# sekelle/SPH-EXA

Hardware: AMD Instinct MI355X
Metric: particle-updates/sec (whole node), Sedov -n 400 and Evrard+gravity -n 200 (higher is better)
Workload: dtype fp64 coordinates + fp32 hydro (reference precision mix); 1 GPU; model=sedov -n 400 --prop ve (64000000 particles), global_batch=64000000, seq_len=1, parallelism=sfc-domain-decomposition x1, ranks=1, backend=none, leaf_capacity=512

## Files before the change

### sphexa_amd/csrc/hip/hydro.hip

```cpp
#include <cfloat>
#include <cstdlib>
#include <type_traits>

#include "common.h"
#include "hip_api.h"
#include "sphx/sph_math.hpp"
#include "staged.h"

namespace sphx::hip
{

#ifndef SPHX_PAIR_BLOCK
#define SPHX_PAIR_BLOCK 256
#endif
constexpr int kBlock = SPHX_PAIR_BLOCK;

template<int B = kBlock>
__device__ __forceinline__ bool targetOf(const NbrArgs& a, int64_t& i, PackedLane& pl, unsigned& n)
{
    __shared__ uint32_t ctabAll[B / 64][kChunkCap];
    unsigned lb     = xcdRemap(blockIdx.x, gridDim.x);
    int64_t t       = int64_t(lb) * B + threadIdx.x;
    i               = a.first + t;
    const int64_t g = t >> 6;
// ... 58 lines not shown
#define SPHX_MOM_BUF 1
#endif
static bool g_kernelFixed = SPHX_KERNEL_FIXED, g_momBuf = SPHX_MOM_BUF;
void setPairPaths(bool kernelFixed, bool momBuf)
{
    g_kernelFixed = kernelFixed;
    g_momBuf      = momBuf;
}

template<class F>
inline void withKf(const SphConsts& sc, F&& f)
{
    if (g_kernelFixed && sc.kernelChoice == 0 && sc.sincIndex == 6.0f) f(std::integral_constant<int, 6>{});
    else f(std::integral_constant<int, 0>{});
}

constexpr int kBufferFormatWord = 0x00020000;

template<class R>
__device__ __forceinline__ CoopLoader<R> coopOf(const R* rec, float4* blockTile, int64_t self, const NbrArgs& a)
{
    return CoopLoader<R>{rec, waveTile<R>(blockTile), unsigned(self)};
}

inline NbrArgs withTot(NbrArgs a, int64_t ntot)
{
    a.ntot = unsigned(ntot);
    return a;
}

inline unsigned gridT(const NbrArgs& a, int block = kBlock) { return gridFor(a.last - a.first, block); }

static int g_pairBlock = kBlock;
#ifndef SPHX_AV_BLOCK
#define SPHX_AV_BLOCK 640
#endif
#ifndef SPHX_GRADH_BLOCK
#define SPHX_GRADH_BLOCK 1024
#endif
#ifndef SPHX_XMASS_BLOCK
#define SPHX_XMASS_BLOCK 1024
#endif
static const unsigned kPairMask = []
{
    const char* e = std::getenv("SPHX_PAIR_MASK");
    return e ? unsigned(std::strtoul(e, nullptr, 0)) : 31u;
}();

void setPairBlock(int block) { g_pairBlock = block == 512 ? 512 : kBlock; }

static unsigned g_staged = []
{
    const char* e = std::getenv("SPHX_STAGED");
    return e ? unsigned(std::strtoul(e, nullptr, 0)) : 12u;
}();

void setStaged(unsigned mask) { g_staged = mask; }
unsigned stagedMask() { return g_staged; }

static bool unionLoopOn(int loop)
{
    const bool big = g_pairBlock == 512 && ((kPairMask >> loop) & 1u);
    return ((g_staged >> loop) & 1u) && (big || (g_staged & 32u));
}

static unsigned* g_stagedCounters = nullptr;
void setStagedCounters(unsigned* counters) { g_stagedCounters = counters; }

#ifndef SPHX_STB_U512
#define SPHX_STB_U512 2264
#endif
#ifndef SPHX_STB_U256
#define SPHX_STB_U256 1128
#endif
template<int B>
constexpr int kUnionCap = B == 512 ? SPHX_STB_U512 : SPHX_STB_U256;
static_assert(sizeof(BlockUnionShared<8, kUnionCap<512>, 2>) * 2 <= 160 * 1024 &&
                  sizeof(BlockUnionShared<4, kUnionCap<256>, 2>) * 4 <= 160 * 1024,
              "16 waves per CU with the unions in LDS");

static bool g_listMasks = false;
void setListMasks(bool on) { g_listMasks = on; }
bool listMasksForced() { return g_listMasks; }
bool listMasksWanted() { return g_listMasks || (g_staged & 1u) || unionLoopOn(2) || unionLoopOn(3); }

inline unsigned gridStaged(const NbrArgs& a) { return unsigned((a.last - a.first + 63) / 64); }

template<class F>
inline void withPairBlock(F&& f, int loop = 0)
{
    if (g_pairBlock == 512 && ((kPairMask >> loop) & 1u)) f(std::integral_constant<int, 512>{});
    else f(std::integral_constant<int, kBlock>{});
}

template<int L, class F>
inline void withPairBlockL(F&& f, int loop)
{
    if (g_pairBlock == 512 && ((kPairMask >> loop) & 1u)) f(std::integral_constant<int, L>{});
    else f(std::integral_constant<int, kBlock>{});
}


__global__ void packPosKernel(int64_t n, const double* __restrict__ x, const double* __restrict__ y,
                              const double* __restrict__ z, const float* __restrict__ m,
                              const float* __restrict__ xm, SrcPos* __restrict__ out)
{
    int64_t i = int64_t(blockIdx.x) * blockDim.x + threadIdx.x;
    if (i >= n) return;
    SrcPos r;
    r.x    = x[i];
    r.y    = y[i];
    r.z    = z[i];
    r.m    = m[i];
    r.xm   = xm ? xm[i] : 0.f;
    out[i] = r;
}

__global__ void packIadKernel(int64_t n, const double* __restrict__ x, const double* __restrict__ y,
                              const double* __restrict__ z, const float* __restrict__ numer,
                              const float* __restrict__ denom, const float* __restrict__ vx,
                              const float* __restrict__ vy, const float* __restrict__ vz,
                              const float* __restrict__ xm, const float* __restrict__ c,
                              const float* __restrict__ divv, SrcIad* __restrict__ out)
{
    int64_t i = int64_t(blockIdx.x) * blockDim.x + threadIdx.x;
    if (i >= n) return;
    SrcIad r;
    r.x    = x[i];
    r.y    = y[i];
    r.z    = z[i];
    r.vol  = numer ? numer[i] / denom[i] : 0.f;
    r.vx   = vx ? vx[i] : 0.f;
    r.vy   = vy ? vy[i] : 0.f;
    r.vz   = vz ? vz[i] : 0.f;
    if (c) r.c = c[i];
    else r.xm = xm ? xm[i] : 0.f;
    r.divv = divv ? divv[i] : 0.f;
// ... 259 lines not shown
    const SrcPosQ pi = ld(unsigned(i));
    const float hi = h[i], hInv = 1.f / hi, h3Inv = hInv * hInv * hInv;
    const float sx = q.inv[0] * 0.25f * hInv, sy = q.inv[1] * 0.25f * hInv, sz = q.inv[2] * 0.25f * hInv;
    float rho0 = 0.f;
    withKernelFn<kKf>(sc, wh, nullptr, [&](const auto& kf) {
        float sum = 0.f;
        forEachNeighbor<SPHX_BATCH_POS>(&pl, 0, n, ld, [&](unsigned, const SrcPosQ& pj) {
            const float ux = float(int32_t(pi.x - pj.x)) * sx;
            const float uy = float(int32_t(pi.y - pj.y)) * sy;
            const float uz = float(int32_t(pi.z - pj.z)) * sz;
            sum += kf.wqIn(sqrtF(ux * ux + uy * uy + uz * uz)) * pj.m;
        });
        rho0 = pi.m + sum / kf.wqScale();
    });
    if (!valid) return;
    const float v = pi.m / (rho0 * float(sc.K) * h3Inv);
    xm[i]         = v;
    if (xmOut) xmOut[i] = SrcXmQ{pi.x, pi.y, pi.z, v};
}

template<int W, int UCAP>
__global__ __launch_bounds__(64 * W) void xmassQStagedKernel(NbrArgs a, SphConsts sc, QFrame q,
                                                             const float* __restrict__ h,
                                                             const SrcPosQ* __restrict__ rec,
                                                             const float* __restrict__ wh, float* __restrict__ xm,
                                                             SrcXmQ* __restrict__ xmOut)
{
    using Ld = StagedLoader<SrcPosQ, W, UCAP>;
    __shared__ typename Ld::Shared sh;
    int64_t i;
    StagedLane sl;
    unsigned n;
    const bool valid = stagedTargetOf<W>(a, i, sl, n);
    const Ld ld{rec, nullptr, 0.f, &sh};
    const KernelFn kf{wh, nullptr, sc.sincIndex, sc.kernelChoice};
    const SrcPosQ pi = ld(unsigned(i));
    const float hi = h[i], hInv = 1.f / hi, h3Inv = hInv * hInv * hInv;
    const float sx = q.inv[0] * 0.25f * hInv, sy = q.inv[1] * 0.25f * hInv, sz = q.inv[2] * 0.25f * hInv;
    float rho0 = 0.f;
    forEachNeighbor<SPHX_BATCH_POS>(&sl, 0, n, ld, [&](unsigned, const SrcPosQ& pj) {
        const float ux = float(int32_t(pi.x - pj.x)) * sx;
        const float uy = float(int32_t(pi.y - pj.y)) * sy;
        const float uz = float(int32_t(pi.z - pj.z)) * sz;
        rho0 += kf.wqIn(sqrtF(ux * ux + uy * uy + uz * uz)) * pj.m;
    });
    reduceAcross(ld, rho0);
    rho0 = pi.m + rho0 / kf.wqScale();
    if (!valid || threadIdx.x >= 64) return;
    const float v = pi.m / (rho0 * float(sc.K) * h3Inv);
    xm[i]         = v;
    if (xmOut) xmOut[i] = SrcXmQ{pi.x, pi.y, pi.z, v};
}

#ifndef SPHX_ST_XMASS_W
#define SPHX_ST_XMASS_W 4
#endif
#ifndef SPHX_ST_XMASS_U
#define SPHX_ST_XMASS_U 1024
#endif

struct EosOut
{
    const double* temp = nullptr;
    float *prho = nullptr, *c = nullptr, *rho = nullptr, *p = nullptr;
};

template<class R, class G, int B = kBlock, int kKf = 0>
__global__ __launch_bounds__(B) void veDefGradhKernel(NbrArgs a, SphConsts sc, G box,
                                                           const float* __restrict__ h, const R* __restrict__ rec,
                                                           const float* __restrict__ wh, const float* __restrict__ whd,
                                                           float* __restrict__ kx, float* __restrict__ gradh,
                                                           float mUniform, const float* __restrict__ vx,
                                                           const float* __restrict__ vy, const float* __restrict__ vz,
                                                           SrcIadQ* __restrict__ iadOut, EosOut eos = EosOut{})
{
    __shared__ float4 tile[B / 64 * 64 * CoopLoader<R>::S];
    int64_t i;
    PackedLane pl;
    unsigned n;
    const bool valid = targetOf<B>(a, i, pl, n);
    float k, g;
    withKernelFn<kKf>(sc, wh, whd, [&](const auto& kf)
                 { veDefGradhJLoop(unsigned(i), sc.K, box, &pl, 0, n, h[i], coopOf(rec, tile, i, a), kf, k, g, mUniform); });
    if (!valid) return;
    kx[i]    = k;
    gradh[i] = g;
    if constexpr (std::is_same_v<R, SrcXmQ>)
    {
        if (iadOut)
        {
            const SrcXmQ pi = rec[i];
            iadOut[i]       = SrcIadQ{pi.x, pi.y, pi.z, pi.xm / k, vx[i], vy[i], vz[i], pi.xm};
        }
        if (eos.temp)
        {
            const float xmi   = rec[i].xm;
            const double rhoi = double(k) * mUniform / xmi;
            double pi, ci;
            idealGasEOS(eos.temp[i], rhoi, sc.muiConst, sc.gamma, pi, ci);
            eos.prho[i] = float(pi / (double(k) * mUniform * mUniform * g));
            eos.c[i]    = float(ci);
            if (eos.rho) eos.rho[i] = float(rhoi);
            if (eos.p) eos.p[i] = float(pi);
        }
    }
}

__global__ void eosVeKernel(int64_t first, int64_t last, SphConsts sc, const double* __restrict__ temp,
                            const float* __restrict__ m, const float* __restrict__ kx, const float* __restrict__ xm,
                            const float* __restrict__ gradh, float* __restrict__ prho, float* __restrict__ c,
                            float* __restrict__ rho, float* __restrict__ p)
{
    int64_t i = first + int64_t(blockIdx.x) * blockDim.x + threadIdx.x;
    if (i >= last) return;
    double rhoi = double(kx[i]) * m[i] / xm[i];
    double pi, ci;
    idealGasEOS(temp[i], rhoi, sc.muiConst, sc.gamma, pi, ci);
    prho[i] = float(pi / (double(kx[i]) * m[i] * m[i] * gradh[i]));
    c[i]    = float(ci);
    if (rho) rho[i] = float(rhoi);
    if (p) p[i] = float(pi);
}

__global__ void eosPolytropicKernel(int64_t first, int64_t last, const float* __restrict__ kx,
                                    const float* __restrict__ xm, const float* __restrict__ m, float* __restrict__ p,
                                    float* __restrict__ c)
{
    int64_t i = first + int64_t(blockIdx.x) * blockDim.x + threadIdx.x;
    if (i >= last) return;
    double rho = double(kx[i]) * m[i] / xm[i], pi, ci;
    polytropicEOS(rho, pi, ci);
    p[i] = float(pi);
    c[i] = float(ci);
}

void eosPolytropic(int64_t first, int64_t last, const float* kx, const float* xm, const float* m, float* p, float* c,
                   hipStream_t s)
{
    if (last <= first) return;
    eosPolytropicKernel<<<gridFor(last - first, 256), 256, 0, s>>>(first, last, kx, xm, m, p, c);
    SPHX_LAUNCH_CHECK();
}

__global__ void eosStdKernel(int64_t first, int64_t last, SphConsts sc, const double* __restrict__ temp,
                             const float* __restrict__ m, float* __restrict__ rho, float* __restrict__ p,
                             float* __restrict__ c)
{
    int64_t i = first + int64_t(blockIdx.x) * blockDim.x + threadIdx.x;
    if (i >= last) return;
    double rhoi = double(m[i]) / rho[i];
    double pi, ci;
    idealGasEOS(temp[i], rhoi, sc.muiConst, sc.gamma, pi, ci);
    rho[i] = float(rhoi);
    p[i]   = float(pi);
    c[i]   = float(ci);
}

struct Six
// ... 638 lines not shown
        double V[3] = {vx[i], vy[i], vz[i]};
        q[0] += 0.5 * mi * (V[0] * V[0] + V[1] * V[1] + V[2] * V[2]);
        if (u) q[1] += u[i] * mi;
        else if (temp) q[1] += cv * temp[i] * mi;
        q[3] += mi * V[0];
        q[4] += mi * V[1];
        q[5] += mi * V[2];
        q[6] += mi * (X[1] * V[2] - X[2] * V[1]);
        q[7] += mi * (X[2] * V[0] - X[0] * V[2]);
        q[8] += mi * (X[0] * V[1] - X[1] * V[0]);
        if (nc) q[9] += double(nc[i]);
    }
    __shared__ double red[4][10];
    int w = threadIdx.x >> 6;
    for (int k = 0; k < 10; ++k)
    {
        double v = waveSum(q[k]);
        if ((threadIdx.x & 63) == 0) red[w][k] = v;
    }
    __syncthreads();
    if (threadIdx.x < 10)
    {
        double s = 0;
        for (int ww = 0; ww < int(blockDim.x >> 6); ++ww)
            s += red[ww][threadIdx.x];
        atomicAdd(&out[threadIdx.x], s);
    }
}


void packPosQ(int64_t n, const double* x, const double* y, const double* z, const float* m, const QFrame& q,
              SrcPosQ* out, hipStream_t s)
{
    if (n <= 0) return;
    packPosQKernel<<<gridFor(n, 256), 256, 0, s>>>(0, n, x, y, z, m, q, out);
    SPHX_LAUNCH_CHECK();
}

void xmass(const NbrArgs& a, const SphConsts& sc, const Box& box, int64_t ntot, const double* x, const double* y,
           const double* z, const float* h, const float* m, const float* wh, void* rec, float* xm, hipStream_t s,
           int inDone, void* xmOut)
{
    if (a.last <= a.first) return;
    if (!sc.fixedPoint)
    {
        packPosKernel<<<gridFor(ntot, 256), 256, 0, s>>>(ntot, x, y, z, m, nullptr, (SrcPos*)rec);
        xmassKernel<<<gridT(a), kBlock, 0, s>>>(withTot(a, ntot), sc, box, h, (const SrcPos*)rec, wh, xm);
    }
    else
    {
        const QFrame q = qframeOf(box, sc.fixedPoint);
        packRanges(inDone, a, ntot, [&](int64_t lo, int64_t hi)
                   { packPosQKernel<<<gridFor(hi - lo, 256), 256, 0, s>>>(lo, hi, x, y, z, m, q, (SrcPosQ*)rec); });
        if (g_staged & 1u)
        {
            xmassQStagedKernel<SPHX_ST_XMASS_W, SPHX_ST_XMASS_U><<<gridStaged(a), 64 * SPHX_ST_XMASS_W, 0, s>>>(
                withTot(a, ntot), sc, q, h, (const SrcPosQ*)rec, wh, xm, (SrcXmQ*)xmOut);
            SPHX_LAUNCH_CHECK();
            return;
        }
        withPairBlockL<SPHX_XMASS_BLOCK>([&](auto bc)
                      {
                          constexpr int B = decltype(bc)::value;
                          withKf(sc, [&](auto kk)
                                 {
                                     xmassQKernel<B, decltype(kk)::value><<<gridT(a, B), B, 0, s>>>(
                                         withTot(a, ntot), sc, q, h, (const SrcPosQ*)rec, wh, xm, (SrcXmQ*)xmOut);
                                 });
                      }, 0);
    }
    SPHX_LAUNCH_CHECK();
}

void veDefGradh(const NbrArgs& a, const SphConsts& sc, const Box& box, int64_t ntot, const double* x,
                const double* y, const double* z, const float* h, const float* m, const float* wh, const float* whd,
                const float* xm, void* rec, float* kx, float* gradh, float mUniform, hipStream_t s, int inDone,
                void* iadOut, const float* vx, const float* vy, const float* vz, const double* eosTemp,
                float* eosPrho, float* eosC, float* eosRho, float* eosP)
{
    if (a.last <= a.first) return;
    if (mUniform > 0.f && sc.fixedPoint)
    {
        const EosOut eos{eosTemp, eosPrho, eosC, eosRho, eosP};
        const QFrame q = qframeOf(box, sc.fixedPoint);
        packRanges(inDone, a, ntot, [&](int64_t lo, int64_t hi)
                   { packXmQKernel<<<gridFor(hi - lo, 256), 256, 0, s>>>(lo, hi, x, y, z, xm, q, (SrcXmQ*)rec); });
        withPairBlockL<SPHX_GRADH_BLOCK>([&](auto bc)
                      {
                          constexpr int B = decltype(bc)::value;
                          withKf(sc, [&](auto kk)
                                 {
                                     veDefGradhKernel<SrcXmQ, QFrame, B, decltype(kk)::value><<<gridT(a, B), B, 0, s>>>(
                                         withTot(a, ntot), sc, q, h, (const SrcXmQ*)rec, wh, whd, kx, gradh, mUniform,
                                         vx, vy, vz, (SrcIadQ*)iadOut, eos);
                                 });
                      }, 1);
    }
    else
    {
        packPosKernel<<<gridFor(ntot, 256), 256, 0, s>>>(ntot, x, y, z, m, xm, (SrcPos*)rec);
        veDefGradhKernel<<<gridT(a), kBlock, 0, s>>>(withTot(a, ntot), sc, box, h, (const SrcPos*)rec, wh, whd, kx,
                                                     gradh, 0.f, vx, vy, vz, nullptr);
        SPHX_LAUNCH_CHECK();
        if (eosTemp) eosVe(a.first, a.last, sc, eosTemp, m, kx, xm, gradh, eosPrho, eosC, eosRho, eosP, s);
    }
    SPHX_LAUNCH_CHECK();
}

void eosVe(int64_t first, int64_t last, const SphConsts& sc, const double* temp, const float* m, const float* kx,
           const float* xm, const float* gradh, float* prho, float* c, float* rho, float* p, hipStream_t s)
{
    if (last <= first) return;
    eosVeKernel<<<gridFor(last - first, 256), 256, 0, s>>>(first, last, sc, temp, m, kx, xm, gradh, prho, c, rho, p);
    SPHX_LAUNCH_CHECK();
}

void eosStd(int64_t first, int64_t last, const SphConsts& sc, const double* temp, const float* m, float* rho,
            float* p, float* c, hipStream_t s)
{
    if (last <= first) return;
    eosStdKernel<<<gridFor(last - first, 256), 256, 0, s>>>(first, last, sc, temp, m, rho, p, c);
    SPHX_LAUNCH_CHECK();
}

void iad(const NbrArgs& a, const SphConsts& sc, const Box& box, int64_t ntot, const double* x, const double* y,
         const double* z, const float* h, const float* wh, const float* numer, const float* denom, void* rec,
         float* const cij[6], hipStream_t s)
{
    if (a.last <= a.first) return;
    packIadKernel<<<gridFor(ntot, 256), 256, 0, s>>>(ntot, x, y, z, numer, denom, nullptr, nullptr, nullptr,
                                                     nullptr, nullptr, nullptr, (SrcIad*)rec);
    Six c;
    for (int k = 0; k < 6; ++k)
        c.p[k] = cij[k];
    iadKernel<<<gridT(a), kBlock, 0, s>>>(withTot(a, ntot), sc, box, h, (const SrcIad*)rec, wh, c);
    SPHX_LAUNCH_CHECK();
}

inline size_t momSideOffset(int64_t ntot) { return (size_t(ntot) * sizeof(SrcMomQ64) + 255) & ~size_t(255); }
// ... 265 lines not shown
```

### sphexa_amd/csrc/hip/staged.h

```cpp
#pragma once

#include "common.h"
#include "sphx/packed_list.hpp"
#include "sphx/sph_math.hpp"

namespace sphx::hip
{

constexpr int kStRows = 64;

template<int UCAP, int RC, bool kSide>
struct StagedShared
{
    float4 rec[UCAP * RC];
    float2 side[kSide ? UCAP : 1];
    uint32_t jl[UCAP];
    uint16_t pos[kStRows * 64];
    uint32_t c0[kStRows];
    uint32_t base[kStRows];
    uint32_t mlo[kStRows], mhi[kStRows];
    int win[2];
};

struct StagedLane
// ... 265 lines not shown
    if constexpr (W > 1)
    {
        float* s            = reinterpret_cast<float*>(ld.sh->rec);
        const unsigned lane = threadIdx.x & 63, w = threadIdx.x >> 6;
        __syncthreads();
        for (int k = 0; k < n; ++k)
            s[(k * W + w) * 64 + lane] = v[k];
        __syncthreads();
        for (int k = 0; k < n; ++k)
        {
            float t = s[(k * W) * 64 + lane];
#pragma unroll
            for (int ww = 1; ww < W; ++ww)
                t += s[(k * W + ww) * 64 + lane];
            v[k] = t;
        }
    }
}

template<class R, int W, int UCAP, bool kSide, class... T>
__device__ void reduceAcrossMax(const StagedLoader<R, W, UCAP, kSide>& ld, T&... v)
{
    if constexpr (W > 1)
    {
        float* s            = reinterpret_cast<float*>(ld.sh->rec);
        const unsigned lane = threadIdx.x & 63, w = threadIdx.x >> 6;
        __syncthreads();
        int k = 0;
        ((s[(k++ * W + w) * 64 + lane] = float(v)), ...);
        __syncthreads();
        k          = 0;
        auto total = [&](int kk)
        {
            float t = s[(kk * W) * 64 + lane];
#pragma unroll
            for (int ww = 1; ww < W; ++ww)
                t = fmaxf(t, s[(kk * W + ww) * 64 + lane]);
            return t;
        };
        ((v = total(k++)), ...);
    }
}


constexpr unsigned kBuSlots = 64;
constexpr uint32_t kBuEmpty = 0xFFFFFFFFu;

struct BlockLane
{
    const int32_t* tab;
    const int32_t* rowsInt;
    unsigned nch, Tc, T;
    unsigned gfirst;

    __device__ __forceinline__ int32_t rowOf(unsigned o) const
    {
        return *(const __attribute__((address_space(4))) int32_t*)(tab + 2 + o);
    }
};

template<int NG, int UCAP, int RC>
struct BlockUnionShared
{
    static constexpr int HS = 64 * NG;
    union
    {
        uint4 rec[(UCAP + 1) * RC];
        uint32_t ctab[NG][kChunkCap];
    };
    uint4 tab[HS];
    uint16_t dense[HS];
    unsigned wsum[NG];
    unsigned fail;
};

template<int B>
__device__ __forceinline__ bool blockTargetOf(const NbrArgs& a, int64_t& i, PackedLane& pl, unsigned& n, BlockLane& bl)
{
    const unsigned lb   = xcdRemap(blockIdx.x, gridDim.x);
    const int64_t t     = int64_t(lb) * B + threadIdx.x;
    i                   = a.first + t;
    const int64_t g     = t >> 6;
    const int64_t G     = (a.last - a.first + 63) / 64;
    const unsigned lane = threadIdx.x & 63;
    bl.tab              = a.nidx + g * int64_t(packedTableInts(a.ngmax));
    bl.rowsInt          = a.nidx + packedTableRegion(G, a.ngmax);
    bl.nch = bl.Tc = bl.T = 0;
    bl.gfirst             = unsigned(a.first + g * 64);
    pl.nblk               = 0;
    if (g < G)
    {
        pl.nblk          = unsigned(*(const __attribute__((address_space(4))) int32_t*)(bl.tab));
        const unsigned w = unsigned(*(const __attribute__((address_space(4))) int32_t*)(bl.tab + 1));
        bl.nch           = min(tableWordNch(w), kChunkCap);
        bl.Tc            = tableWordTc(w);
        bl.T             = tableWordT(w);
    }
    pl.tab  = bl.tab + 2 + bl.T;
    pl.rows = reinterpret_cast<const int4*>(bl.rowsInt) + lane;
    pl.ctab = nullptr;
#ifdef SPHX_DEVICE_CHECKS
    pl.ntot = a.ntot;
    SPHX_DCHECK(pl.nblk <= listBlocksMax(a.ngmax), 1);
    pl.nblk = min(pl.nblk, listBlocksMax(a.ngmax));
#endif
    if (i >= a.last)
    {
        i       = a.last - 1;
        pl.self = unsigned(i);
        n       = 0;
        return false;
    }
    pl.self = unsigned(i);
    const int cnt = a.nc[i] - 1;
    n             = unsigned(cnt < 0 ? 0 : (unsigned(cnt) < a.ngmax ? cnt : a.ngmax));
    return true;
}

template<int NG, int UCAP, int RC>
__device__ __forceinline__ void loadChunkTable(const BlockLane& bl, PackedLane& pl, BlockUnionShared<NG, UCAP, RC>& sh)
{
    const unsigned lane = threadIdx.x & 63;
    uint32_t* ctab      = sh.ctab[threadIdx.x >> 6];
    for (unsigned e = lane; e < bl.nch; e += 64)
        ctab[e] = uint32_t(bl.rowsInt[size_t(bl.rowOf(e >> 8)) * 256 + (e & 255)]);
    asm volatile("s_waitcnt vmcnt(0) lgkmcnt(0)" ::: "memory");
    pl.ctab = ctab;
}

template<class R, int NG, int UCAP>
__device__ bool stageBlockUnion(const BlockLane& bl, const R* __restrict__ rec, unsigned ntot,
                                BlockUnionShared<NG, UCAP, int(sizeof(R) / 16)>& sh, unsigned* counters)
{
    constexpr int RC = int(sizeof(R) / 16);
    constexpr int HS = 64 * NG;
    static_assert((HS & (HS - 1)) == 0, "hash size is a power of two");
    static_assert(UCAP + 64 < 65536 && NG * (kBuSlots - 1) * 64 < 65536, "the scan packs two 16-bit counts");
    const unsigned t = threadIdx.x, lane = t & 63, wave = t >> 6;
    sh.tab[t] = make_uint4(kBuEmpty, 0u, 0u, 0u);
    if (t == 0) sh.fail = 0u;
    __syncthreads();
    const bool masks  = bl.T >= bl.Tc + maskTabRows(bl.nch) && bl.T > bl.Tc;
    const bool waveOk = bl.nch <= kBuSlots && (bl.nch <= 1u || masks);
    const bool mine   = waveOk && lane >= 1u && lane < bl.nch;
    bool bad          = !waveOk;
    unsigned e        = 0;
    if (mine)
    {
        const uint32_t cb = uint32_t(bl.rowsInt[size_t(bl.rowOf(0)) * 256 + lane]);
        const int32_t* mr = bl.rowsInt + size_t(bl.rowOf(bl.Tc)) * 256 + 2 * lane;
        uint32_t lo = uint32_t(mr[0]), hi = uint32_t(mr[1]);
        if (cb >= ntot) bad = true;
        else
        {
            const unsigned avail = min(ntot - cb, 64u);
            const uint64_t keep  = avail >= 64u ? ~0ull : ((1ull << avail) - 1ull);
            lo &= uint32_t(keep);
            hi &= uint32_t(keep >> 32);
            unsigned hsh = (cb * 2654435761u) >> (32 - __builtin_ctz(unsigned(HS)));
            bool done    = false;
            for (int tries = 0; tries < HS && !done; ++tries)
            {
                const uint32_t old = atomicCAS(&sh.tab[hsh].x, kBuEmpty, cb);
                if (old == kBuEmpty || old == cb)
                {
                    if (lo) atomicOr(&sh.tab[hsh].z, lo);
                    if (hi) atomicOr(&sh.tab[hsh].w, hi);
                    e    = hsh;
                    done = true;
                }
                else hsh = (hsh + 1u) & unsigned(HS - 1);
            }
            if (!done) bad = true;
        }
    }
    if (bad) sh.fail = 1u;
    __syncthreads();
    uint4 ent          = sh.tab[t];
    const bool used    = ent.x != kBuEmpty;
    const unsigned cnt = used ? unsigned(__popc(ent.z) + __popc(ent.w)) : 0u;
    const unsigned pk  = cnt | (used ? 1u << 16 : 0u);
    unsigned incl      = pk;
#pragma unroll
    for (int o = 1; o < 64; o <<= 1)
    {
        const unsigned up = unsigned(__shfl_up(int(incl), o));
        if (int(lane) >= o) incl += up;
    }
    if (lane == 63) sh.wsum[wave] = incl;
    __syncthreads();
    unsigned before = 0, total = 0;
#pragma unroll
    for (int w = 0; w < NG; ++w)
    {
        const unsigned s = sh.wsum[w];
        before += unsigned(w) < wave ? s : 0u;
        total += s;
    }
    const unsigned excl = before + incl - pk;
    const unsigned nrec = total & 0xFFFFu, nent = total >> 16;
    const bool staged   = sh.fail == 0u && nrec <= unsigned(UCAP);
    if (counters && t == 0) atomicAdd(&counters[staged ? 0 : 1], 1u);
    if (!staged)
    {
        __syncthreads();
        return false;
    }
    if (used)
    {
        sh.tab[t].y               = excl & 0xFFFFu;
        sh.dense[excl >> 16]      = uint16_t(t);
    }
    __syncthreads();
    uint4 slotEnt = make_uint4(bl.gfirst, 0u, 0u, 0u);
    if (mine) slotEnt = sh.tab[e];
    for (unsigned k = wave; k < nent; k += NG)
    {
        const uint4 en   = sh.tab[sh.dense[k]];
        const uint64_t m = uint64_t(en.w) << 32 | en.z;
        if ((m >> lane) & 1)
        {
            const unsigned p = en.y + unsigned(__popcll(m & lanemaskLt()));
            const uint4* src = reinterpret_cast<const uint4*>(rec) + size_t(en.x + lane) * RC;
#pragma unroll
            for (int c = 0; c < RC; ++c)
                sh.rec[p * RC + c] = src[c];
        }
    }
    __syncthreads();
    sh.tab[t] = slotEnt;
    __syncthreads();
    return true;
}

template<class R, int NG, int UCAP, class F>
__device__ void forEachNeighborUnion(const PackedLane& pl, const BlockLane& bl,
                                     const BlockUnionShared<NG, UCAP, int(sizeof(R) / 16)>& sh, F&& f)
{
    constexpr int RC    = int(sizeof(R) / 16);
    const unsigned nblk = pl.nblk;
    if (nblk == 0) return;
    const uint4* wtab = sh.tab + (threadIdx.x >> 6) * 64;
    int4 w            = pl.block(0);
    auto batch = [&](int w0, int w1)
    {
        const uint32_t ws[2] = {uint32_t(w0), uint32_t(w1)};
        unsigned j[4];
        R rr[4];
#pragma unroll
        for (int u = 0; u < 4; ++u)
        {
            const uint32_t code = (ws[u >> 1] >> ((u & 1) * 16)) & 0xFFFFu;
            const unsigned slot = code & (kBuSlots - 1u), off = code >> kChunkSlotBits;
            const uint4 en      = wtab[slot];
            const uint32_t below = (1u << (off & 31u)) - 1u;
            const bool upper     = off >= 32u;
            const uint32_t lo = upper ? en.z : en.z & below, hi = upper ? en.w & below : 0u;
            unsigned p        = en.y + unsigned(__popc(lo)) + unsigned(__popc(hi));
            j[u]              = en.x + off;
#ifdef SPHX_DEVICE_CHECKS
            const bool ok = (code & kChunkSlotMask) < max(bl.nch, 1u) && p < unsigned(UCAP) &&
                            ((code & kChunkSlotMask) != 0u || j[u] == pl.self);
            SPHX_DCHECK(ok, 0);
            if (!ok)
            {
                p    = 0u;
                j[u] = pl.self;
            }
#endif
            uint4 o4[RC];
#pragma unroll
            for (int c = 0; c < RC; ++c)
                o4[c] = sh.rec[p * RC + c];
            float4 o[RC];
#pragma unroll
            for (int c = 0; c < RC; ++c)
                o[c] = make_float4(__uint_as_float(o4[c].x), __uint_as_float(o4[c].y), __uint_as_float(o4[c].z),
                                   __uint_as_float(o4[c].w));
            rr[u] = stagedUnpack<R>(o);
        }
#pragma unroll
        for (int u = 0; u < 4; ++u)
        {
            pinRegs(rr[u]);
            if (j[u] != pl.self) f(j[u], rr[u]);
        }
    };
    for (unsigned b = 0; b < nblk; ++b)
    {
        const int4 wn = pl.block(b + 1);
        batch(w.x, w.y);
        batch(w.z, w.w);
        w = wn;
    }
    (void)bl;
}

template<class R, int NG, int UCAP>
struct BlockUnionLoader
{
    using Shared = BlockUnionShared<NG, UCAP, int(sizeof(R) / 16)>;
    const R* r;
    const Shared* sh;
    const BlockLane* bl;
    bool staged;

    __device__ R operator()(unsigned j) const { return r[j]; }
};

template<int B, class R, int NG, int UCAP, class F>
__device__ void forEachNeighbor(const PackedLane* pl, int, unsigned, const BlockUnionLoader<R, NG, UCAP>& ld, F&& f)
{
    if (ld.staged) forEachNeighborUnion<R, NG, UCAP>(*pl, *ld.bl, *ld.sh, f);
    else forEachNeighborDirect(*pl, ld, f);
}

}
```

### sphexa_amd/csrc/include/sphx/sph_math.hpp

```cpp
#pragma once

#include <cmath>
#include <cstddef>
#include <cstdint>

#include "annotation.hpp"
#include "box.hpp"
#include "packed_list.hpp"

namespace sphx
{

#ifndef SPHX_HYDRO_TYPE
#define SPHX_HYDRO_TYPE float
#endif
using HT = SPHX_HYDRO_TYPE;
constexpr bool kHydroF32 = sizeof(HT) == 4;
using CT = double;

constexpr int kTableSize = 20000;

struct SphConsts
{
    double K;
// ... 975 lines not shown
template<class Ld, class... T>
SPHX_HD void reduceAcrossMax(const Ld&, T&...)
{
}
template<class Ld>
SPHX_HD void reduceAcrossN(const Ld&, HT*, int)
{
}

template<class Idx, class Ld, class KF>
SPHX_HD HT xmassJLoop(unsigned i, double K, const Box& box, const Idx* nbr, int stride, unsigned nc, HT hi,
                      const Ld& ld, const KF& kf)
{
    SrcPos pi = ld(i);
    HT hInv = HT(1) / hi, h3Inv = hInv * hInv * hInv, hq = HT(0.25) * hInv;
    HT rho0 = 0;
    forEachNeighbor<SPHX_BATCH_POS>(nbr, stride, nc, ld, [&](unsigned j, const SrcPos& pj) {
        HT rx, ry, rz;
        pairDelta(pi.x, pi.y, pi.z, pj.x, pj.y, pj.z, hi, box, rx, ry, rz);
        HT dist = sqrtF(rx * rx + ry * ry + rz * rz);
        rho0 += kf.wqIn(dist * hq) * pj.m;
    });
    rho0 = pi.m + rho0 / kf.wqScale();
    return pi.m / (rho0 * HT(K) * h3Inv);
}

template<class G, class Idx, class Ld, class KF>
SPHX_HD void veDefGradhJLoop(unsigned i, double K, const G& box, const Idx* nbr, int stride, unsigned nc, HT hi,
                             const Ld& ld, const KF& kf, HT& kxOut, HT& gradhOut,
                             HT mUniform = HT(0))
{
    const auto pi = ld(i);
    HT mi = massOf(pi, mUniform), xmi = pi.xm;
    HT hInv = HT(1) / hi, h3Inv = hInv * hInv * hInv, hq = HT(0.25) * hInv;

    HT kxi      = 0;
    HT whomegai = 0;
    HT wrho0i   = 0;
    const auto bx = vgprFrame(box);
    forEachNeighbor<SPHX_BATCH_POS>(nbr, stride, nc, ld, [&](unsigned j, const auto& pj) {
        HT rx, ry, rz;
        pairSep(bx, pi, pj, hi, rx, ry, rz);
        HT dist  = sqrtF(rx * rx + ry * ry + rz * rz);
        HT w, vdw;
        kf.wdq(dist * hq, w, vdw);
        HT dterh = -(HT(3) * w + vdw);
        HT xmj   = pj.xm;
        kxi += w * xmj;
        whomegai += dterh * xmj;
        wrho0i += dterh * massOf(pj, mUniform);
    });
    reduceAcross(ld, kxi, whomegai, wrho0i);
    const HT invS = HT(1) / kf.wqScale();
    kxi      = xmi + kxi * invS;
    whomegai = -HT(3) * xmi + whomegai * invS;
    wrho0i   = -HT(3) * mi + wrho0i * invS;
    HT Kf = HT(K);
    kxi *= Kf * h3Inv;
    whomegai *= Kf * h3Inv * hInv;
    wrho0i *= Kf * h3Inv * hInv;

    whomegai  = whomegai * mi / xmi + (kxi - Kf * xmi * h3Inv) * wrho0i;
    HT rhoi   = kxi * mi / xmi;
    HT dhdrho = -hi / (rhoi * HT(3));
    kxOut     = kxi;
    gradhOut  = HT(1) - dhdrho * whomegai;
}

SPHX_HD void invertTau(HT tau[6], HT hi, double K, HT c[6])
{
    auto getExp = [](HT v) { return v == HT(0) ? 0 : ilogb(v); };
    int expSum  = getExp(tau[0]) + getExp(tau[1]) + getExp(tau[2]) + getExp(tau[3]) + getExp(tau[4]) + getExp(tau[5]);
    HT norm     = ldexp(HT(1), -expSum / 6);
    for (int k = 0; k < 6; ++k)
        tau[k] *= norm;
    HT t11 = tau[0], t12 = tau[1], t13 = tau[2], t22 = tau[3], t23 = tau[4], t33 = tau[5];
    HT det = t11 * t22 * t33 + HT(2) * t12 * t23 * t13 - t11 * t23 * t23 - t22 * t13 * t13 - t33 * t12 * t12;
    HT factor = norm * (hi * hi * hi) / (det * HT(K));
    c[0]      = (t22 * t33 - t23 * t23) * factor;
    c[1]      = (t13 * t23 - t33 * t12) * factor;
    c[2]      = (t12 * t23 - t22 * t13) * factor;
    c[3]      = (t11 * t33 - t13 * t13) * factor;
    c[4]      = (t13 * t12 - t11 * t23) * factor;
    c[5]      = (t11 * t22 - t12 * t12) * factor;
}

template<class Idx, class Ld>
SPHX_HD void iadJLoop(unsigned i, double K, const Box& box, const Idx* nbr, int stride, unsigned nc, HT hi,
                      const Ld& ld, const KernelFn& kf, HT c[6])
{
    HT tau[6] = {0, 0, 0, 0, 0, 0};
    SrcIad pi = ld(i);
    HT hq     = HT(0.25) / hi;
    forEachNeighbor<SPHX_BATCH_IAD>(nbr, stride, nc, ld, [&](unsigned j, const SrcIad& pj) {
        HT rx, ry, rz;
        pairDelta(pi.x, pi.y, pi.z, pj.x, pj.y, pj.z, hi, box, rx, ry, rz);
        HT dist = sqrtF(rx * rx + ry * ry + rz * rz);
        HT w    = kf.wqIn(dist * hq);
        HT vw   = pj.vol * w;
        tau[0] += rx * rx * vw;
        tau[1] += rx * ry * vw;
        tau[2] += rx * rz * vw;
        tau[3] += ry * ry * vw;
        tau[4] += ry * rz * vw;
        tau[5] += rz * rz * vw;
    });
    const HT invS = HT(1) / kf.wqScale();
    for (int k = 0; k < 6; ++k)
        tau[k] *= invS;
// ... 555 lines not shown
```

Measured before the change: 611.9 million particle-updates/s.

## Stage block-union neighbor records in LDS for xmass and gradh loops

Adds block-union LDS-staged variants of the xmass and VE gradh kernels and enables them by default through new staged mask bits. The union table now stores precomputed byte offsets, so each neighbor lookup costs one popcount and a shift instead of split-mask arithmetic. Self-exclusion now compares against a precomputed self address in LDS. It also pins intermediate registers in the Sinc6 gradh epilogue. The aim is to replace global or cooperative record loads with shared-memory reuse, at the price of large LDS footprints, 1024-thread blocks that may lower occupancy, and a fallback path whenever the union overflows.

After: 625.6 million particle-updates/s, median of 6. 1.02x the previous value.

```diff
diff --git a/sphexa_amd/csrc/hip/hydro.hip b/sphexa_amd/csrc/hip/hydro.hip
--- a/sphexa_amd/csrc/hip/hydro.hip
+++ b/sphexa_amd/csrc/hip/hydro.hip
@@ -134,7 +134,7 @@
 static unsigned g_staged = []
 {
     const char* e = std::getenv("SPHX_STAGED");
-    return e ? unsigned(std::strtoul(e, nullptr, 0)) : 12u;
+    return e ? unsigned(std::strtoul(e, nullptr, 0)) : 78u;
 }();
 
 void setStaged(unsigned mask) { g_staged = mask; }
@@ -142,8 +142,9 @@
 
 static bool unionLoopOn(int loop)
 {
-    const bool big = g_pairBlock == 512 && ((kPairMask >> loop) & 1u);
-    return ((g_staged >> loop) & 1u) && (big || (g_staged & 32u));
+    const bool big     = g_pairBlock == 512 && ((kPairMask >> loop) & 1u);
+    const unsigned bit = loop == 0 ? 6u : unsigned(loop);
+    return ((g_staged >> bit) & 1u) && (big || (g_staged & 32u));
 }
 
 static unsigned* g_stagedCounters = nullptr;
@@ -161,10 +162,46 @@
                   sizeof(BlockUnionShared<4, kUnionCap<256>, 2>) * 4 <= 160 * 1024,
               "16 waves per CU with the unions in LDS");
 
+#ifndef SPHX_STB_XG_U1024
+#define SPHX_STB_XG_U1024 3900
+#endif
+#ifndef SPHX_STB_XG_U512
+#define SPHX_STB_XG_U512 2704
+#endif
+#ifndef SPHX_STB_XG_U256
+#define SPHX_STB_XG_U256 2260
+#endif
+#ifndef SPHX_STB_XG_BLOCK
+#define SPHX_STB_XG_BLOCK 1024
+#endif
+template<int B>
+constexpr int kUnionCapXg = B == 1024 ? SPHX_STB_XG_U1024 : B == 512 ? SPHX_STB_XG_U512 : SPHX_STB_XG_U256;
+static_assert(sizeof(BlockUnionShared<16, kUnionCapXg<1024>, 1>) * 2 <= 160 * 1024 &&
+                  sizeof(BlockUnionShared<8, kUnionCapXg<512>, 1>) * 3 <= 160 * 1024 &&
+                  sizeof(BlockUnionShared<4, kUnionCapXg<256>, 1>) * 4 <= 160 * 1024,
+              "blocks per CU with the 16-B unions in LDS");
+static const int kXgBlock = []
+{
+    const char* e = std::getenv("SPHX_STB_XG_BLOCK");
+    return (e ? std::atoi(e) : SPHX_STB_XG_BLOCK) == 512 ? 512 : 1024;
+}();
+
+template<class F>
+inline void withXgBlock(F&& f, int loop)
+{
+    const bool big = g_pairBlock == 512 && ((kPairMask >> loop) & 1u);
+    if (!big) f(std::integral_constant<int, kBlock>{});
+    else if (kXgBlock == 512) f(std::integral_constant<int, 512>{});
+    else f(std::integral_constant<int, 1024>{});
+}
+
 static bool g_listMasks = false;
 void setListMasks(bool on) { g_listMasks = on; }
 bool listMasksForced() { return g_listMasks; }
-bool listMasksWanted() { return g_listMasks || (g_staged & 1u) || unionLoopOn(2) || unionLoopOn(3); }
+bool listMasksWanted()
+{
+    return g_listMasks || (g_staged & 1u) || unionLoopOn(0) || unionLoopOn(1) || unionLoopOn(2) || unionLoopOn(3);
+}
 
 inline unsigned gridStaged(const NbrArgs& a) { return unsigned((a.last - a.first + 63) / 64); }
 
@@ -530,6 +567,41 @@
     if (xmOut) xmOut[i] = SrcXmQ{pi.x, pi.y, pi.z, v};
 }
 
+template<int B, int kKf, int UCAP>
+__global__ __launch_bounds__(B) __attribute__((amdgpu_waves_per_eu(B == 1024 ? 8 : 4))) void xmassQUnionKernel(
+    NbrArgs a, SphConsts sc, QFrame q, const float* __restrict__ h, const SrcPosQ* __restrict__ rec,
+    const float* __restrict__ wh, float* __restrict__ xm, SrcXmQ* __restrict__ xmOut, unsigned* counters)
+{
+    using Ld = BlockUnionLoader<SrcPosQ, B / 64, UCAP>;
+    __shared__ typename Ld::Shared sh;
+    int64_t i;
+    PackedLane pl;
+    BlockLane bl;
+    unsigned n;
+    const bool valid  = blockTargetOf<B>(a, i, pl, n, bl);
+    const bool staged = stageBlockUnion<SrcPosQ, B / 64, UCAP>(bl, rec, a.ntot, sh, counters);
+    if (!staged) loadChunkTable(bl, pl, sh);
+    const Ld ld{rec, &sh, &bl, staged};
+    const SrcPosQ pi = ld(unsigned(i));
+    const float hi = h[i], hInv = 1.f / hi, h3Inv = hInv * hInv * hInv;
+    const float sx = q.inv[0] * 0.25f * hInv, sy = q.inv[1] * 0.25f * hInv, sz = q.inv[2] * 0.25f * hInv;
+    float rho0 = 0.f;
+    withKernelFn<kKf>(sc, wh, nullptr, [&](const auto& kf) {
+        float sum = 0.f;
+        forEachNeighbor<SPHX_BATCH_POS>(&pl, 0, n, ld, [&](unsigned, const SrcPosQ& pj) {
+            const float ux = float(int32_t(pi.x - pj.x)) * sx;
+            const float uy = float(int32_t(pi.y - pj.y)) * sy;
+            const float uz = float(int32_t(pi.z - pj.z)) * sz;
+            sum += kf.wqIn(sqrtF(ux * ux + uy * uy + uz * uz)) * pj.m;
+        });
+        rho0 = pi.m + sum / kf.wqScale();
+    });
+    if (!valid) return;
+    const float v = pi.m / (rho0 * float(sc.K) * h3Inv);
+    xm[i]         = v;
+    if (xmOut) xmOut[i] = SrcXmQ{pi.x, pi.y, pi.z, v};
+}
+
 #ifndef SPHX_ST_XMASS_W
 #define SPHX_ST_XMASS_W 4
 #endif
@@ -543,24 +615,13 @@
     float *prho = nullptr, *c = nullptr, *rho = nullptr, *p = nullptr;
 };
 
-template<class R, class G, int B = kBlock, int kKf = 0>
-__global__ __launch_bounds__(B) void veDefGradhKernel(NbrArgs a, SphConsts sc, G box,
-                                                           const float* __restrict__ h, const R* __restrict__ rec,
-                                                           const float* __restrict__ wh, const float* __restrict__ whd,
-                                                           float* __restrict__ kx, float* __restrict__ gradh,
-                                                           float mUniform, const float* __restrict__ vx,
-                                                           const float* __restrict__ vy, const float* __restrict__ vz,
-                                                           SrcIadQ* __restrict__ iadOut, EosOut eos = EosOut{})
-{
-    __shared__ float4 tile[B / 64 * 64 * CoopLoader<R>::S];
-    int64_t i;
-    PackedLane pl;
-    unsigned n;
-    const bool valid = targetOf<B>(a, i, pl, n);
-    float k, g;
-    withKernelFn<kKf>(sc, wh, whd, [&](const auto& kf)
-                 { veDefGradhJLoop(unsigned(i), sc.K, box, &pl, 0, n, h[i], coopOf(rec, tile, i, a), kf, k, g, mUniform); });
-    if (!valid) return;
+template<class R>
+__device__ __forceinline__ void gradhEpilogue(int64_t i, const SphConsts& sc, const R* __restrict__ rec, float k,
+                                              float g, float* __restrict__ kx, float* __restrict__ gradh,
+                                              float mUniform, const float* __restrict__ vx,
+                                              const float* __restrict__ vy, const float* __restrict__ vz,
+                                              SrcIadQ* __restrict__ iadOut, const EosOut& eos)
+{
     kx[i]    = k;
     gradh[i] = g;
     if constexpr (std::is_same_v<R, SrcXmQ>)
@@ -582,6 +643,50 @@
             if (eos.p) eos.p[i] = float(pi);
         }
     }
+}
+
+template<class R, class G, int B = kBlock, int kKf = 0>
+__global__ __launch_bounds__(B) void veDefGradhKernel(NbrArgs a, SphConsts sc, G box,
+                                                           const float* __restrict__ h, const R* __restrict__ rec,
+                                                           const float* __restrict__ wh, const float* __restrict__ whd,
+                                                           float* __restrict__ kx, float* __restrict__ gradh,
+                                                           float mUniform, const float* __restrict__ vx,
+                                                           const float* __restrict__ vy, const float* __restrict__ vz,
+                                                           SrcIadQ* __restrict__ iadOut, EosOut eos = EosOut{})
+{
+    __shared__ float4 tile[B / 64 * 64 * CoopLoader<R>::S];
+    int64_t i;
+    PackedLane pl;
+    unsigned n;
+    const bool valid = targetOf<B>(a, i, pl, n);
+    float k, g;
+    withKernelFn<kKf>(sc, wh, whd, [&](const auto& kf)
+                 { veDefGradhJLoop(unsigned(i), sc.K, box, &pl, 0, n, h[i], coopOf(rec, tile, i, a), kf, k, g, mUniform); });
+    if (!valid) return;
+    gradhEpilogue(i, sc, rec, k, g, kx, gradh, mUniform, vx, vy, vz, iadOut, eos);
+}
+
+template<int B, int kKf, int UCAP>
+__global__ __launch_bounds__(B) __attribute__((amdgpu_waves_per_eu(B == 1024 ? 8 : 4))) void veDefGradhUnionKernel(
+    NbrArgs a, SphConsts sc, QFrame box, const float* __restrict__ h, const SrcXmQ* __restrict__ rec,
+    const float* __restrict__ wh, const float* __restrict__ whd, float* __restrict__ kx, float* __restrict__ gradh,
+    float mUniform, const float* __restrict__ vx, const float* __restrict__ vy, const float* __restrict__ vz,
+    SrcIadQ* __restrict__ iadOut, EosOut eos, unsigned* counters)
+{
+    using Ld = BlockUnionLoader<SrcXmQ, B / 64, UCAP>;
+    __shared__ typename Ld::Shared sh;
+    int64_t i;
+    PackedLane pl;
+    BlockLane bl;
+    unsigned n;
+    const bool valid  = blockTargetOf<B>(a, i, pl, n, bl);
+    const bool staged = stageBlockUnion<SrcXmQ, B / 64, UCAP>(bl, rec, a.ntot, sh, counters);
+    if (!staged) loadChunkTable(bl, pl, sh);
+    float k, g;
+    withKernelFn<kKf>(sc, wh, whd, [&](const auto& kf)
+                 { veDefGradhJLoop(unsigned(i), sc.K, box, &pl, 0, n, h[i], Ld{rec, &sh, &bl, staged}, kf, k, g, mUniform); });
+    if (!valid) return;
+    gradhEpilogue(i, sc, rec, k, g, kx, gradh, mUniform, vx, vy, vz, iadOut, eos);
 }
 
 __global__ void eosVeKernel(int64_t first, int64_t last, SphConsts sc, const double* __restrict__ temp,
@@ -1326,6 +1431,21 @@
         const QFrame q = qframeOf(box, sc.fixedPoint);
         packRanges(inDone, a, ntot, [&](int64_t lo, int64_t hi)
                    { packPosQKernel<<<gridFor(hi - lo, 256), 256, 0, s>>>(lo, hi, x, y, z, m, q, (SrcPosQ*)rec); });
+        if (unionLoopOn(0))
+        {
+            withXgBlock([&](auto bc)
+                        {
+                            constexpr int B = decltype(bc)::value;
+                            withKf(sc, [&](auto kk)
+                                   {
+                                       xmassQUnionKernel<B, decltype(kk)::value, kUnionCapXg<B>>
+                                           <<<gridT(a, B), B, 0, s>>>(withTot(a, ntot), sc, q, h, (const SrcPosQ*)rec, wh,
+                                                                      xm, (SrcXmQ*)xmOut, g_stagedCounters);
+                                   });
+                        }, 0);
+            SPHX_LAUNCH_CHECK();
+            return;
+        }
         if (g_staged & 1u)
         {
             xmassQStagedKernel<SPHX_ST_XMASS_W, SPHX_ST_XMASS_U><<<gridStaged(a), 64 * SPHX_ST_XMASS_W, 0, s>>>(
@@ -1359,6 +1479,23 @@
         const QFrame q = qframeOf(box, sc.fixedPoint);
         packRanges(inDone, a, ntot, [&](int64_t lo, int64_t hi)
                    { packXmQKernel<<<gridFor(hi - lo, 256), 256, 0, s>>>(lo, hi, x, y, z, xm, q, (SrcXmQ*)rec); });
+        if (unionLoopOn(1))
+        {
+            withXgBlock([&](auto bc)
+                        {
+                            withKf(sc, [&](auto kk)
+                                   {
+                                       constexpr int KK = decltype(kk)::value, B0 = decltype(bc)::value;
+                                       constexpr int B  = KK == 0 && B0 == 1024 ? 512 : B0;
+                                       veDefGradhUnionKernel<B, KK, kUnionCapXg<B>>
+                                           <<<gridT(a, B), B, 0, s>>>(withTot(a, ntot), sc, q, h, (const SrcXmQ*)rec, wh,
+                                                                      whd, kx, gradh, mUniform, vx, vy, vz,
+                                                                      (SrcIadQ*)iadOut, eos, g_stagedCounters);
+                                   });
+                        }, 1);
+            SPHX_LAUNCH_CHECK();
+            return;
+        }
         withPairBlockL<SPHX_GRADH_BLOCK>([&](auto bc)
                       {
                           constexpr int B = decltype(bc)::value;
diff --git a/sphexa_amd/csrc/hip/staged.h b/sphexa_amd/csrc/hip/staged.h
--- a/sphexa_amd/csrc/hip/staged.h
+++ b/sphexa_amd/csrc/hip/staged.h
@@ -341,6 +341,7 @@
     const int32_t* rowsInt;
     unsigned nch, Tc, T;
     unsigned gfirst;
+    unsigned selfAddr;
 
     __device__ __forceinline__ int32_t rowOf(unsigned o) const
     {
@@ -376,6 +377,7 @@
     bl.rowsInt          = a.nidx + packedTableRegion(G, a.ngmax);
     bl.nch = bl.Tc = bl.T = 0;
     bl.gfirst             = unsigned(a.first + g * 64);
+    bl.selfAddr           = 0;
     pl.nblk               = 0;
     if (g < G)
     {
@@ -393,6 +395,7 @@
     SPHX_DCHECK(pl.nblk <= listBlocksMax(a.ngmax), 1);
     pl.nblk = min(pl.nblk, listBlocksMax(a.ngmax));
 #endif
+    if (pl.nblk == 0) bl.nch = 0;
     if (i >= a.last)
     {
         i       = a.last - 1;
@@ -418,7 +421,7 @@
 }
 
 template<class R, int NG, int UCAP>
-__device__ bool stageBlockUnion(const BlockLane& bl, const R* __restrict__ rec, unsigned ntot,
+__device__ bool stageBlockUnion(BlockLane& bl, const R* __restrict__ rec, unsigned ntot,
                                 BlockUnionShared<NG, UCAP, int(sizeof(R) / 16)>& sh, unsigned* counters)
 {
     constexpr int RC = int(sizeof(R) / 16);
@@ -488,10 +491,10 @@
     }
     const unsigned excl = before + incl - pk;
     const unsigned nrec = total & 0xFFFFu, nent = total >> 16;
-    const bool staged   = sh.fail == 0u && nrec <= unsigned(UCAP);
-    if (counters && t == 0) atomicAdd(&counters[staged ? 0 : 1], 1u);
-    if (!staged)
-    {
+    const bool fits     = sh.fail == 0u && nrec <= unsigned(UCAP);
+    if (!fits)
+    {
+        if (counters && t == 0) atomicAdd(&counters[1], 1u);
         __syncthreads();
         return false;
     }
@@ -501,8 +504,27 @@
         sh.dense[excl >> 16]      = uint16_t(t);
     }
     __syncthreads();
-    uint4 slotEnt = make_uint4(bl.gfirst, 0u, 0u, 0u);
+    constexpr unsigned RS    = unsigned(RC) * 16u;
+    constexpr unsigned spare = unsigned(UCAP) * RS;
+    uint4 slotEnt = make_uint4(0u, 0u, 0u, 0u);
     if (mine) slotEnt = sh.tab[e];
+    unsigned selfAddr = spare, found = 0;
+    for (uint64_t ov = ballot(mine && slotEnt.x + 64u > bl.gfirst && slotEnt.x < bl.gfirst + 64u); ov; ov &= ov - 1)
+    {
+        const int s       = __builtin_ctzll(ov);
+        const unsigned c0 = unsigned(__builtin_amdgcn_readlane(int(slotEnt.x), s));
+        const unsigned b  = unsigned(__builtin_amdgcn_readlane(int(slotEnt.y), s));
+        const uint64_t m  = uint64_t(unsigned(__builtin_amdgcn_readlane(int(slotEnt.w), s))) << 32 |
+                           unsigned(__builtin_amdgcn_readlane(int(slotEnt.z), s));
+        const unsigned d  = bl.gfirst + lane - c0;
+        if (d < 64u && ((m >> d) & 1))
+        {
+            selfAddr = (b + unsigned(__popcll(m & ((1ull << d) - 1ull)))) * RS;
+            ++found;
+        }
+    }
+    bl.selfAddr = selfAddr;
+    if (found > 1u) sh.fail = 1u;
     for (unsigned k = wave; k < nent; k += NG)
     {
         const uint4 en   = sh.tab[sh.dense[k]];
@@ -517,7 +539,12 @@
         }
     }
     __syncthreads();
-    sh.tab[t] = slotEnt;
+    const bool staged = sh.fail == 0u;
+    if (counters && t == 0) atomicAdd(&counters[staged ? 0 : 1], 1u);
+    __syncthreads();
+    if (!staged) return false;
+    sh.tab[t] = mine ? make_uint4(slotEnt.y * RS, slotEnt.z, (slotEnt.y + unsigned(__popc(slotEnt.z))) * RS, slotEnt.w)
+                     : make_uint4(spare, 0u, spare, 0u);
     __syncthreads();
     return true;
 }
@@ -531,36 +558,36 @@
     if (nblk == 0) return;
     const uint4* wtab = sh.tab + (threadIdx.x >> 6) * 64;
     int4 w            = pl.block(0);
+    constexpr unsigned RS = unsigned(RC) * 16u, spare = unsigned(UCAP) * RS;
+    const char* recs      = reinterpret_cast<const char*>(sh.rec);
+    const unsigned self   = bl.selfAddr;
     auto batch = [&](int w0, int w1)
     {
         const uint32_t ws[2] = {uint32_t(w0), uint32_t(w1)};
-        unsigned j[4];
+        unsigned a[4];
         R rr[4];
 #pragma unroll
         for (int u = 0; u < 4; ++u)
         {
-            const uint32_t code = (ws[u >> 1] >> ((u & 1) * 16)) & 0xFFFFu;
-            const unsigned slot = code & (kBuSlots - 1u), off = code >> kChunkSlotBits;
+            const uint32_t wd   = ws[u >> 1];
+            const bool hiHalf   = u & 1;
+            const unsigned slot = (hiHalf ? wd >> 16 : wd) & (kBuSlots - 1u);
+            const unsigned sh5  = (hiHalf ? wd >> 26 : wd >> kChunkSlotBits) & 31u;
+            const bool upper    = hiHalf ? int32_t(wd) < 0 : (wd & 0x8000u) != 0u;
             const uint4 en      = wtab[slot];
-            const uint32_t below = (1u << (off & 31u)) - 1u;
-            const bool upper     = off >= 32u;
-            const uint32_t lo = upper ? en.z : en.z & below, hi = upper ? en.w & below : 0u;
-            unsigned p        = en.y + unsigned(__popc(lo)) + unsigned(__popc(hi));
-            j[u]              = en.x + off;
+            const uint32_t m    = (upper ? en.w : en.y) & ~(~0u << sh5);
+            a[u]                = (upper ? en.z : en.x) + unsigned(__popc(m)) * RS;
 #ifdef SPHX_DEVICE_CHECKS
-            const bool ok = (code & kChunkSlotMask) < max(bl.nch, 1u) && p < unsigned(UCAP) &&
-                            ((code & kChunkSlotMask) != 0u || j[u] == pl.self);
+            const unsigned code = (hiHalf ? wd >> 16 : wd) & 0xFFFFu;
+            const bool ok       = (code & kChunkSlotMask) < max(bl.nch, 1u) && a[u] <= spare &&
+                            ((code & kChunkSlotMask) != 0u || a[u] == spare);
             SPHX_DCHECK(ok, 0);
-            if (!ok)
-            {
-                p    = 0u;
-                j[u] = pl.self;
-            }
+            if (!ok) a[u] = spare;
 #endif
             uint4 o4[RC];
 #pragma unroll
             for (int c = 0; c < RC; ++c)
-                o4[c] = sh.rec[p * RC + c];
+                o4[c] = *reinterpret_cast<const uint4*>(recs + a[u] + c * 16);
             float4 o[RC];
 #pragma unroll
             for (int c = 0; c < RC; ++c)
@@ -572,7 +599,7 @@
         for (int u = 0; u < 4; ++u)
         {
             pinRegs(rr[u]);
-            if (j[u] != pl.self) f(j[u], rr[u]);
+            if (a[u] != self && a[u] != spare) f(pl.self, rr[u]);
         }
     };
     for (unsigned b = 0; b < nblk; ++b)
@@ -582,7 +609,6 @@
         batch(w.z, w.w);
         w = wn;
     }
-    (void)bl;
 }
 
 template<class R, int NG, int UCAP>
diff --git a/sphexa_amd/csrc/include/sphx/sph_math.hpp b/sphexa_amd/csrc/include/sphx/sph_math.hpp
--- a/sphexa_amd/csrc/include/sphx/sph_math.hpp
+++ b/sphexa_amd/csrc/include/sphx/sph_math.hpp
@@ -1051,9 +1051,24 @@
     });
     reduceAcross(ld, kxi, whomegai, wrho0i);
     const HT invS = HT(1) / kf.wqScale();
-    kxi      = xmi + kxi * invS;
-    whomegai = -HT(3) * xmi + whomegai * invS;
-    wrho0i   = -HT(3) * mi + wrho0i * invS;
+#if defined(__HIP_DEVICE_COMPILE__)
+    if constexpr (std::is_same_v<KF, KernelFnSinc6> && std::is_same_v<HT, float>)
+    {
+        HT sk = kxi * invS, sw = whomegai * invS, sr = wrho0i * invS;
+        pinRegs(sk);
+        pinRegs(sw);
+        pinRegs(sr);
+        kxi      = xmi + sk;
+        whomegai = fmaf(-HT(3), xmi, sw);
+        wrho0i   = fmaf(-HT(3), mi, sr);
+    }
+    else
+#endif
+    {
+        kxi      = xmi + kxi * invS;
+        whomegai = -HT(3) * xmi + whomegai * invS;
+        wrho0i   = -HT(3) * mi + wrho0i * invS;
+    }
     HT Kf = HT(K);
     kxi *= Kf * h3Inv;
     whomegai *= Kf * h3Inv * hInv;
```
